# XiSHEN0220/RANSAC-Flow

Measured on NVIDIA H100. Metric: image-pairs/sec at 480x640, nbIter=1k RANSAC, higher is better.
Workload: dtype f32-grade: fp16 hi/lo split operands and activations (22 significand bits), 3 wgmma MMAs per MAC, fp32 accumulate; fp16-split correlation; fp32/fp64 RANSAC

## Files before the change

### ransac-flow_b200/csrc/gemm_tc.cu

```cuda
#include <cuda.h>
#include <cuda_fp16.h>

#include <climits>
#include <mutex>
#include <unordered_map>

#include "common.cuh"
#include "tc_common.cuh"

namespace rf {

constexpr int K_TF32 = 0, K_F16 = 1, K_SPLIT = 2, K_TF32X3 = 3;
constexpr int MODE_CONV = 0, MODE_CORR = 1;
constexpr int O_F32 = 0, O_F16 = 1, O_SPLIT = 2;
constexpr int WG_THREADS = 288;

struct alignas(64) WgParams {
    CUtensorMap mapA[RF_MAX_IMGS];
    CUtensorMap mapA2[RF_MAX_IMGS];
    CUtensorMap mapY[RF_MAX_IMGS];
    CUtensorMap mapR[RF_MAX_IMGS];
    CUtensorMap mapB;
    CUtensorMap mapBlo;
    int nimg;
    int ntiles;
    int tile_start[RF_MAX_IMGS + 1];
    int tiles_x[RF_MAX_IMGS];
    int tw[RF_MAX_IMGS];
// ... 2 lines not shown
    int R, S, pad, stride, Cin, Cout, relu, round_out;
    int dil;
    int kc1, stride2;
    long long plane;
    const float* bias;
    const void* residual;
    void* y;
    unsigned long long* rowbest;
    unsigned long long* colbest;
    int NA, NB;
};
static_assert(sizeof(WgParams) <= 32764, "kernel parameter space (CUDA 12.1+ large kernel parameters)");

template <int KIND, int BN, int MODE>
struct WgCfg {
    static constexpr int NPL = (KIND == K_SPLIT || KIND == K_TF32X3) ? 2 : 1;
    static constexpr int A_BYTES = NPL * TC_A_BYTES;
    static constexpr int B_PLANE = BN * 128;
    static constexpr int STAGE_BYTES = A_BYTES + NPL * B_PLANE;
    static constexpr bool ONE_CTA = MODE == MODE_CORR || NPL * BN >= 256;
    static constexpr int BUDGET = ONE_CTA ? 200 * 1024 : 100 * 1024;
    static constexpr int STAGES = BUDGET / STAGE_BYTES > 6 ? 6 : BUDGET / STAGE_BYTES;
    static constexpr int CTAS_PER_SM = ONE_CTA ? 1 : 2;
    static constexpr int SMEM_BYTES = STAGES * STAGE_BYTES + 1024  + 256 ;
    static_assert(STAGES >= 2 && SMEM_BYTES <= 227 * 1024, "shared memory");
};

__device__ __forceinline__ __half2 pack_sat(float a, float b) {
    uint32_t r;
    asm("cvt.rn.satfinite.f16x2.f32 %0, %1, %2;" : "=r"(r) : "f"(b), "f"(a));
    return *reinterpret_cast<__half2*>(&r);
}
__device__ __forceinline__ void split2(float a, float b, __half2& hi, __half2& lo) {
    hi = pack_sat(a, b);
    const float2 f = __half22float2(hi);
    lo = pack_sat((a - f.x) * 2048.f, (b - f.y) * 2048.f);
}

template <int KIND, int BN, int NACC>
__device__ __forceinline__ void mma_block(float (&acc)[NACC][BN / 2], uint32_t sa, uint32_t sb) {
// ... 1 lines not shown
#pragma unroll
    for (int k = 0; k < 4; ++k) {
        const uint64_t ah = wg_desc(sa + 32 * k), bh = wg_desc(sb + 32 * k);
        if constexpr (KIND == K_SPLIT || KIND == K_TF32X3) {
            const uint64_t al = wg_desc(sa + TC_A_BYTES + 32 * k), bl = wg_desc(sb + BN * 128 + 32 * k);
            float (&x)[BN / 2] = acc[NACC - 1];
            wgmma<TF32, BN>(x, al, bh);
            wgmma<TF32, BN>(x, ah, bl);
            wgmma<TF32, BN>(acc[0], ah, bh);
        } else {
            wgmma<TF32, BN>(acc[0], ah, bh);
        }
    }
}

template <int KIND, int BN, int MODE, int OUT>
__global__ void __launch_bounds__(WG_THREADS, WgCfg<KIND, BN, MODE>::CTAS_PER_SM)
wg_kernel(const __grid_constant__ WgParams p) {
    using Cfg = WgCfg<KIND, BN, MODE>;
    constexpr int STAGES = Cfg::STAGES;
    constexpr int BK = (KIND == K_TF32 || KIND == K_TF32X3) ? TC_BK : TC_BK_F16;
    constexpr int NACC = KIND == K_SPLIT ? 2 : 1;
    constexpr bool SLOT = MODE == MODE_CONV && OUT != O_F32;
    constexpr int BOX_BYTES = (OUT == O_SPLIT ? 2 : 1) * 128 * 128;
    static_assert(!SLOT || (BN / 64) * BOX_BYTES <= Cfg::STAGE_BYTES, "the output tile fits one stage");
    extern __shared__ uint8_t smem_raw[];
    uint8_t* smem = smem_raw + ((1024u - (smem_u32(smem_raw) & 1023u)) & 1023u);
    uint64_t* full = reinterpret_cast<uint64_t*>(smem + STAGES * Cfg::STAGE_BYTES);
    uint64_t* empty = full + STAGES;
    const int warp = threadIdx.x >> 5, lane = threadIdx.x & 31;
    const int kc = p.Cin / BK;
    const int KI = p.R * p.S * kc;

    const int t_first = MODE == MODE_CORR ? 0 : (int)blockIdx.x;
    const int t_step = MODE == MODE_CORR ? 1 : (int)gridDim.x;
    const int t_end = MODE == MODE_CORR ? 1 : p.ntiles;
    const int nt = (p.Cout + BN - 1) / BN;
    struct Tile { int img, tw, ox0, oy0, n0; };
    auto decode = [&](int t) {
        const int mtile = MODE == MODE_CORR ? (int)blockIdx.y : t / nt;
        const int ntile = MODE == MODE_CORR ? (int)blockIdx.x : t - mtile * nt;
        Tile T;
        T.img = 0;
#pragma unroll
        for (int j = 1; j < RF_MAX_IMGS; ++j) T.img += (j < p.nimg && mtile >= p.tile_start[j]) ? 1 : 0;
        const int tloc = mtile - p.tile_start[T.img];
        T.tw = p.tw[T.img];
        const int tyi = tloc / p.tiles_x[T.img], txi = tloc - tyi * p.tiles_x[T.img];
        T.ox0 = txi * T.tw;
        T.oy0 = tyi * (128 / T.tw);
        T.n0 = ntile * BN;
        return T;
    };
    auto boxes = [&](const Tile& T) { return BN == 64 || T.n0 + 64 >= p.Cout ? 1 : 2; };

    if (threadIdx.x == 0) {
        for (int s = 0; s < STAGES; ++s) { mbar_init(&full[s], 1); mbar_init(&empty[s], 256); }
        fence_barrier_init();
    }
    __syncthreads();

    if (warp == 8) {
        if (lane == 0) {
            tma_prefetch_desc(&p.mapB);
            uint32_t prefetched = 0;
            int st = 0;
            uint32_t ph = 0;
            for (int t = t_first; t < t_end; t += t_step) {
                const Tile T = decode(t);
                if (!((prefetched >> T.img) & 1u)) {
                    prefetched |= 1u << T.img;
                    tma_prefetch_desc(&p.mapA[T.img]);
                    if constexpr (SLOT) {
                        tma_prefetch_desc(&p.mapY[T.img]);
                        if (p.residual) tma_prefetch_desc(&p.mapR[T.img]);
                    }
                }
                for (int it = 0; it < KI; ++it) {
                    mbar_wait(&empty[st], ph ^ 1);
                    uint8_t* sa = smem + st * Cfg::STAGE_BYTES;
                    uint8_t* sb = sa + Cfg::A_BYTES;
                    mbar_expect_tx(&full[st], Cfg::STAGE_BYTES);
                    if constexpr (MODE == MODE_CORR) {
                        const int c0 = it * BK;
                        tma_load_3d(sa, &p.mapA[0], &full[st], c0, T.ox0, 0);
                        tma_load_3d(sa + TC_A_BYTES, &p.mapA2[0], &full[st], c0, T.ox0, 0);
                        tma_load_2d(sb, &p.mapB, &full[st], c0, T.n0);
                        tma_load_2d(sb + Cfg::B_PLANE, &p.mapBlo, &full[st], c0, T.n0);
                    } else {
                        const int tap = it / kc, cc = it - tap * kc;
                        const int r = tap / p.S, s = tap - r * p.S;
                        const int c0 = cc * BK, x = T.ox0 * p.stride + s * p.dil - p.pad, y = T.oy0 * p.stride + r * p.dil - p.pad;
                        const int kcol = tap * p.Cin + c0;
                        if constexpr (KIND == K_SPLIT) {
                            if (cc < p.kc1) tma_load_4d(sa, &p.mapA[T.img], &full[st], c0, x, y, 0);
                            else tma_load_4d(sa, &p.mapA2[T.img], &full[st], (cc - p.kc1) * BK, T.ox0 * p.stride2, T.oy0 * p.stride2, 0);
                            tma_load_3d(sb, &p.mapB, &full[st], kcol, T.n0, 0);
                        } else {
                            tma_load_3d(sa, &p.mapA[T.img], &full[st], c0, x, y);
                            tma_load_2d(sb, &p.mapB, &full[st], kcol, T.n0);
                        }
                    }
                    if (++st == STAGES) { st = 0; ph ^= 1; }
                }
                if constexpr (SLOT) {
                    mbar_wait(&empty[st], ph ^ 1);
                    if (p.residual) {
                        const int nb = boxes(T);
                        uint8_t* slot = smem + st * Cfg::STAGE_BYTES;
                        mbar_expect_tx(&full[st], nb * BOX_BYTES);
                        for (int b = 0; b < nb; ++b) {
                            if constexpr (OUT == O_SPLIT) tma_load_4d(slot + b * BOX_BYTES, &p.mapR[T.img], &full[st], T.n0 + 64 * b, T.ox0, T.oy0, 0);
                            else tma_load_3d(slot + b * BOX_BYTES, &p.mapR[T.img], &full[st], T.n0 + 64 * b, T.ox0, T.oy0);
                        }
                    } else {
                        mbar_arrive(&full[st]);
                    }
                    if (++st == STAGES) { st = 0; ph ^= 1; }
                }
            }
        }
        return;
    }

    const int g = warp >> 2;
    const int rbase = 64 * g + 16 * (warp & 3) + (lane >> 2);
    const int cbase = 2 * (lane & 3);
    auto before = [](int s) { return s == 0 ? STAGES - 1 : s - 1; };
    int st = 0;
    uint32_t ph = 0;
    bool stored = false;
    for (int t = t_first; t < t_end; t += t_step) {
        const Tile T = decode(t);
        float acc[NACC][BN / 2];
#pragma unroll
        for (int a = 0; a < NACC; ++a)
#pragma unroll
            for (int i = 0; i < BN / 2; ++i) acc[a][i] = 0.f;
        for (int it = 0; it < KI; ++it) {
            mbar_wait(&full[st], ph);
            const uint32_t sa = smem_u32(smem + st * Cfg::STAGE_BYTES);
            wg_fence();
            mma_block<KIND, BN, NACC>(acc, sa + g * (64 * 128), sa + Cfg::A_BYTES);
            wg_commit();
            wg_wait<1>();
            if (it > 0) {
                mbar_arrive(&empty[before(st)]);
            } else if (SLOT && stored) {
                if (threadIdx.x == 0) bulk_wait_read();
                mbar_arrive(&empty[before(st)]);
            }
            if (++st == STAGES) { st = 0; ph ^= 1; }
        }
        wg_wait<0>();
#pragma unroll
        for (int a = 0; a < NACC; ++a) wg_fence_regs(acc[a]);
        mbar_arrive(&empty[before(st)]);

        auto value = [&](int i) -> float {
            if constexpr (KIND == K_SPLIT) return fmaf(acc[1][i], 0.00048828125f, acc[0][i]);
            else return acc[0][i];
        };

        if constexpr (SLOT) {
            mbar_wait(&full[st], ph);
            uint8_t* slot = smem + st * Cfg::STAGE_BYTES;
#pragma unroll
            for (int h = 0; h < 2; ++h) {
                const int m = rbase + 8 * h;
#pragma unroll
                for (int j = 0; j < BN / 8; ++j) {
                    const int c = 8 * j + cbase, n = T.n0 + c;
                    if (n >= p.Cout) continue;
                    float v0 = value(4 * j + 2 * h), v1 = value(4 * j + 2 * h + 1);
                    if (p.bias) { v0 += __ldg(p.bias + n); v1 += __ldg(p.bias + n + 1); }
                    uint8_t* e = slot + (c >> 6) * BOX_BYTES + m * 128 + ((((c & 63) >> 3) ^ (m & 7)) << 4) + (c & 7) * 2;
                    if (p.residual) {
                        if constexpr (OUT == O_F16) {
                            const float2 r = __half22float2(*reinterpret_cast<const __half2*>(e));
                            v0 += r.x; v1 += r.y;
                        } else {
// ... 12 lines not shown
                        *reinterpret_cast<__half2*>(e + 128 * 128) = lo;
                    }
                }
            }
            fence_proxy_async();
            asm volatile("bar.sync 1, 256;" ::: "memory");
            if (threadIdx.x == 0) {
                const int nb = boxes(T);
                for (int b = 0; b < nb; ++b) {
                    if constexpr (OUT == O_SPLIT) tma_store_4d(&p.mapY[T.img], slot + b * BOX_BYTES, T.n0 + 64 * b, T.ox0, T.oy0, 0);
                    else tma_store_3d(&p.mapY[T.img], slot + b * BOX_BYTES, T.n0 + 64 * b, T.ox0, T.oy0);
                }
                bulk_commit();
            }
            stored = true;
            if (++st == STAGES) { st = 0; ph ^= 1; }
        } else if constexpr (MODE == MODE_CONV) {
            const int img = T.img, tw = T.tw;
#pragma unroll
            for (int h = 0; h < 2; ++h) {
                const int m = rbase + 8 * h;
                const int py = m / tw, px = m - py * tw;
                const int oy = T.oy0 + py, ox = T.ox0 + px;
                if (oy >= p.Ho[img] || ox >= p.Wo[img]) continue;
                const long long pix = p.out_pix[img] + (long long)oy * p.Wo[img] + ox;
#pragma unroll
                for (int j = 0; j < BN / 8; ++j) {
                    const int n = T.n0 + 8 * j + cbase;
                    if (n >= p.Cout) continue;
                    const bool two = n + 1 < p.Cout;
                    float v0 = value(4 * j + 2 * h), v1 = value(4 * j + 2 * h + 1);
                    if (p.bias) { v0 += __ldg(p.bias + n); if (two) v1 += __ldg(p.bias + n + 1); }
// ... 103 lines not shown
    int Hs[RF_MAX_IMGS], Ws[RF_MAX_IMGS];
    int Ho[RF_MAX_IMGS], Wo[RF_MAX_IMGS];
    long long in_pix[RF_MAX_IMGS], out_pix[RF_MAX_IMGS];
    long long plane;
    const float* x;
    const float* bias;
    __half* y;
};

__device__ __forceinline__ uint32_t stem_pack_split(float v) {
    __half2 hi, lo;
    split2(v, 0.f, hi, lo);
    return (*reinterpret_cast<uint32_t*>(&hi) & 0xFFFFu) | (*reinterpret_cast<uint32_t*>(&lo) << 16);
}

struct StemFrag { uint32_t h[4], l[4]; };

template <int KK, int j>
__device__ __forceinline__ void stem_gather(StemFrag& f, const uint32_t* __restrict__ w, int base, const int4* sK, int q) {
    const int4 o4 = sK[j * 4 + q];
    const int o[4] = {o4.x, o4.y, o4.z, o4.w};
    uint32_t v[2][4];
#pragma unroll
    for (int h = 0; h < 2; ++h)
#pragma unroll
        for (int e = 0; e < 4; ++e) v[h][e] = (16 * (j + 1) <= KK || o[e] >= 0) ? w[base + 24 * h + o[e]] : 0u;
#pragma unroll
    for (int e = 0; e < 2; ++e)
#pragma unroll
        for (int h = 0; h < 2; ++h) {
            f.h[2 * e + h] = __byte_perm(v[h][2 * e], v[h][2 * e + 1], 0x5410);
            f.l[2 * e + h] = __byte_perm(v[h][2 * e], v[h][2 * e + 1], 0x7632);
        }
}

template <int KK, int KSTEPS, bool SPLIT, int j, int NACC>
__device__ __forceinline__ void stem_mma(float (&acc)[NACC][32], StemFrag (&buf)[2], const uint32_t* w, int base, const int4* sK, int q,
                                         uint32_t sB) {
    if constexpr (j < KSTEPS) {
        constexpr int NPL = SPLIT ? 2 : 1;
        StemFrag& f = buf[j & 1];
        wg_fence();
        const uint32_t b = sB + (j >> 2) * NPL * ST_B_PLANE + 32 * (j & 3);
        const uint64_t bh = wg_desc(b);
        if constexpr (SPLIT) {
            wgmma_f16_n64_rs(acc[1], f.l, bh);
            wgmma_f16_n64_rs(acc[1], f.h, wg_desc(b + ST_B_PLANE));
        }
        wgmma_f16_n64_rs(acc[0], f.h, bh);
        wg_commit();
        if constexpr (j + 1 < KSTEPS) {
            wg_wait<1>();
            stem_gather<KK, j + 1>(buf[(j + 1) & 1], w, base, sK, q);
        }
        stem_mma<KK, KSTEPS, SPLIT, j + 1>(acc, buf, w, base, sK, q, sB);
    }
// ... 83 lines not shown
    stage_window(sIn);
    __syncthreads();

    const int q = lane & 3;
    const int rbase = 64 * g + 16 * (warp & 3) + (lane >> 2), cbase = 2 * q;
    const int base = (rbase >> 5) * S * G::LD + 3 * (rbase & 31);
    const uint32_t sB32 = smem_u32(sB);
    int wb = 0, tb = 0;
    for (bool first = true; u < u_end; ++u, first = false) {
        const uint32_t* w = sIn + wb * G::WIN;
        float acc[NACC][32];
#pragma unroll
        for (int a = 0; a < NACC; ++a)
#pragma unroll
            for (int i = 0; i < 32; ++i) acc[a][i] = 0.f;
        StemFrag frag[2];
        stem_gather<G::KK, 0>(frag[0], w, base, sK, q);
        if (first) mbar_wait(bar_b, 0);
        stem_mma<G::KK, G::KSTEPS, SPLIT, 0>(acc, frag, w, base, sK, q, sB32);
        const bool more = u + 1 < u_end;
        Unit N = U;
        if (more) {
            N = decode(u + 1);
            load_window(N);
        }
        wg_wait<0>();
#pragma unroll
        for (int a = 0; a < NACC; ++a) wg_fence_regs(acc[a]);

        const int img = U.img;
        uint8_t* tile = sT + tb * ST_T_BYTES;
// ... 184 lines not shown
    return get_map4(out, ptr, d0, d1, d2, 0, 0, b0, b1, b2, 0, es_, esize);
}

int pick_tw(int Ho, int Wo) {
    int best = 16;
    long long best_area = -1;
    const int cands[5] = {16, 32, 8, 64, 128};
    for (int i = 0; i < 5; ++i) {
        int tw = cands[i], th = 128 / tw;
        long long area = (long long)((Wo + tw - 1) / tw) * ((Ho + th - 1) / th);
        if (best_area < 0 || area < best_area) { best_area = area; best = tw; }
    }
    return best;
}

template <int KIND, int BN, int MODE, int OUT>
static int launch_wg(const WgParams& p, dim3 grid, cudaStream_t st) {
    using Cfg = WgCfg<KIND, BN, MODE>;
    static bool attr[64] = {false};
    const int dev = current_device();
    if (!attr[dev]) {
        RF_CUDA(cudaFuncSetAttribute(wg_kernel<KIND, BN, MODE, OUT>, cudaFuncAttributeMaxDynamicSharedMemorySize, Cfg::SMEM_BYTES));
        attr[dev] = true;
    }
    wg_kernel<KIND, BN, MODE, OUT><<<grid, WG_THREADS, Cfg::SMEM_BYTES, st>>>(p);
    RF_LAUNCHED();
    return 0;
}

template <int KIND, int BN, int OUT>
static int launch_conv_bn(const WgParams& p, cudaStream_t st) {
    const int resident = WgCfg<KIND, BN, MODE_CONV>::CTAS_PER_SM * num_sms();
    return launch_wg<KIND, BN, MODE_CONV, OUT>(p, dim3(p.ntiles < resident ? p.ntiles : resident), st);
}
template <int KIND, int OUT>
static int launch_conv(const WgParams& p, int BN, cudaStream_t st) {
    return BN == 128 ? launch_conv_bn<KIND, 128, OUT>(p, st) : launch_conv_bn<KIND, 64, OUT>(p, st);
}

struct SplitDual { const void* x2; const int* hw2; int Cin2, stride2; };

static int conv_impl(const ImgSet& batch, const ConvParams& cp, const void* w, cudaStream_t st, int kind, bool out32, const SplitDual* dual) {
    const bool flat = cp.R == 1 && cp.S == 1 && cp.stride == 1 && cp.pad == 0 && (dual == nullptr || dual->stride2 == 1);
    int hw_flat[2] = {1, 0};
    ImgSet flat_set;
    if (flat) {
        RF_REQUIRE(batch.out_pix[batch.n] <= INT_MAX, "rf_conv2d_nhwc: more than 2^31 - 1 pixels in one batch");
        hw_flat[1] = (int)batch.out_pix[batch.n];
        RF_REQUIRE(make_imgset(flat_set, 1, hw_flat, 1, 1, 0) == 0, "rf_conv2d_nhwc: bad image set");
    }
    const ImgSet& set = flat ? flat_set : batch;
    const int* hw2 = dual == nullptr ? nullptr : flat ? hw_flat : dual->hw2;
    WgParams p;
    memset(&p, 0, sizeof(p));
    const bool split = kind == K_SPLIT;
    const unsigned esz = kind == K_TF32 ? 4u : 2u;
    const unsigned bk = kind == K_TF32 ? TC_BK : TC_BK_F16;
    const int BN = cp.Cout > 64 ? 128 : 64;
    const char* xb = reinterpret_cast<const char*>(cp.x);
    const unsigned long long in_plane = (unsigned long long)set.in_pix[set.n] * cp.Cin * 2ull;
    long long in2_pix[RF_MAX_IMGS + 1] = {0};
    if (dual)
        for (int i = 0; i < set.n; ++i) in2_pix[i + 1] = in2_pix[i] + (long long)hw2[2 * i] * hw2[2 * i + 1];
    const unsigned long long in2_plane = dual ? (unsigned long long)in2_pix[set.n] * dual->Cin2 * 2ull : 0ull;
    p.nimg = set.n;
    const bool tma_out = kind != K_TF32 && !out32;
    const unsigned long long out_plane = (unsigned long long)set.out_pix[set.n] * cp.Cout * 2ull;
    const char* yb = reinterpret_cast<const char*>(cp.y);
    const char* rb = reinterpret_cast<const char*>(cp.residual);
    int tiles = 0;
    for (int i = 0; i < set.n; ++i) {
        const int tw = flat ? 128 : pick_tw(set.Ho[i], set.Wo[i]), th = 128 / tw;
        p.tw[i] = tw;
        p.tiles_x[i] = (set.Wo[i] + tw - 1) / tw;
        p.tile_start[i] = tiles;
        tiles += p.tiles_x[i] * ((set.Ho[i] + th - 1) / th);
        p.Ho[i] = set.Ho[i]; p.Wo[i] = set.Wo[i];
        p.out_pix[i] = set.out_pix[i];
        int rc = split ? get_map4(&p.mapA[i], xb + set.in_pix[i] * cp.Cin * 2, (unsigned long long)cp.Cin, (unsigned long long)set.W[i],
                                  (unsigned long long)set.H[i], 2, in_plane, bk, (unsigned)tw, (unsigned)th, 2, (unsigned)cp.stride, 2)
                       : get_map(&p.mapA[i], xb + set.in_pix[i] * cp.Cin * esz, (unsigned long long)cp.Cin, (unsigned long long)set.W[i],
                                 (unsigned long long)set.H[i], bk, (unsigned)tw, (unsigned)th, (unsigned)cp.stride, esz);
        if (!rc && dual)
            rc = get_map4(&p.mapA2[i], static_cast<const char*>(dual->x2) + in2_pix[i] * dual->Cin2 * 2, (unsigned long long)dual->Cin2,
                          (unsigned long long)hw2[2 * i + 1], (unsigned long long)hw2[2 * i], 2, in2_plane, bk, (unsigned)tw,
                          (unsigned)th, 2, (unsigned)dual->stride2, 2);
        const long long o = set.out_pix[i] * cp.Cout * 2;
        for (int m = 0; m < (cp.residual ? 2 : 1) && tma_out && !rc; ++m) {
            CUtensorMap* map = m == 0 ? &p.mapY[i] : &p.mapR[i];
            const void* base = (m == 0 ? yb : rb) + o;
            rc = split ? get_map4(map, base, (unsigned long long)cp.Cout, (unsigned long long)set.Wo[i], (unsigned long long)set.Ho[i], 2,
                                  out_plane, 64, (unsigned)tw, (unsigned)th, 2, 1, 2)
                       : get_map(map, base, (unsigned long long)cp.Cout, (unsigned long long)set.Wo[i], (unsigned long long)set.Ho[i],
                                 64, (unsigned)tw, (unsigned)th, 1, 2);
        }
        if (rc) return rc;
    }
    RF_REQUIRE(tiles > 0, "rf_conv2d_nhwc: empty output");
    for (int i = set.n; i <= RF_MAX_IMGS; ++i) p.tile_start[i] = tiles;
    p.out_pix[set.n] = set.out_pix[set.n];
    int rc = split ? get_map(&p.mapB, w, (unsigned long long)cp.K, (unsigned long long)cp.Cout, 2, bk, (unsigned)BN, 2, 1, 2)
                   : get_map(&p.mapB, w, (unsigned long long)cp.K, (unsigned long long)cp.Cout, 0, bk, (unsigned)BN, 0, 1, esz);
    if (rc) return rc;
    p.R = cp.R; p.S = cp.S; p.pad = cp.pad; p.stride = cp.stride; p.Cin = cp.Cin; p.Cout = cp.Cout; p.relu = cp.relu; p.round_out = cp.round_out;
    p.dil = cp.dil;
    p.kc1 = cp.Cin / (int)bk;
    p.stride2 = 1;
    if (dual) { p.Cin = cp.Cin + dual->Cin2; p.stride2 = dual->stride2; }
    p.plane = (long long)set.out_pix[set.n] * cp.Cout;
    p.bias = cp.bias; p.residual = cp.residual; p.y = cp.y;
    p.ntiles = tiles * ((cp.Cout + BN - 1) / BN);
    if (kind == K_TF32) return launch_conv<K_TF32, O_F32>(p, BN, st);
    if (kind == K_F16) return out32 ? launch_conv<K_F16, O_F32>(p, BN, st) : launch_conv<K_F16, O_F16>(p, BN, st);
    return out32 ? launch_conv<K_SPLIT, O_F32>(p, BN, st) : launch_conv<K_SPLIT, O_SPLIT>(p, BN, st);
}

template <int KS, int S, bool SPLIT>
static int stem_impl(const float* x, int nimg, const int* hw_host, const void* w, const float* bias, void* y, int pool, void* stream) {
    using G = StemGeo<KS, S>;
    RF_REQUIRE(x != nullptr && w != nullptr && y != nullptr, "rf_stem: null pointer");
    RF_REQUIRE(((uintptr_t)y % 16) == 0 && ((uintptr_t)w % 16) == 0, "rf_stem: pointers must be 16-byte aligned");
    ImgSet set;
    RF_REQUIRE(make_imgset(set, nimg, hw_host, KS, S, G::PAD) == 0, "rf_stem: bad image set");
    StemParams p;
    memset(&p, 0, sizeof(p));
    p.nimg = nimg;
    p.pool = pool ? 1 : 0;
    int units = 0;
    long long out = 0;
// ... 155 lines not shown
```

### ransac-flow_b200/csrc/tc_common.cuh

```cuda
#pragma once
#include <cuda.h>
#include <cuda_fp16.h>

#include "common.cuh"
#include "wgmma.cuh"

namespace rf {

constexpr int TC_BK = 32;
constexpr int TC_BK_F16 = 64;
constexpr int TC_A_BYTES = 128 * 128;


__device__ __forceinline__ uint32_t smem_u32(const void* p) { return (uint32_t)__cvta_generic_to_shared(p); }

__device__ __forceinline__ void mbar_init(uint64_t* bar, uint32_t count) {
    asm volatile("mbarrier.init.shared::cta.b64 [%0], %1;" ::"r"(smem_u32(bar)), "r"(count));
}
__device__ __forceinline__ void mbar_expect_tx(uint64_t* bar, uint32_t bytes) {
    asm volatile("mbarrier.arrive.expect_tx.shared::cta.b64 _, [%0], %1;" ::"r"(smem_u32(bar)), "r"(bytes) : "memory");
}
__device__ __forceinline__ void mbar_arrive(uint64_t* bar) {
    asm volatile("mbarrier.arrive.shared::cta.b64 _, [%0];" ::"r"(smem_u32(bar)) : "memory");
}
// ... 36 lines not shown
__device__ __forceinline__ void bulk_commit() { asm volatile("cp.async.bulk.commit_group;" ::: "memory"); }
__device__ __forceinline__ void bulk_wait_read() { asm volatile("cp.async.bulk.wait_group.read 0;" ::: "memory"); }
__device__ __forceinline__ void bulk_wait() { asm volatile("cp.async.bulk.wait_group 0;" ::: "memory"); }
__device__ __forceinline__ void tma_prefetch_desc(const CUtensorMap* map) {
    asm volatile("prefetch.tensormap [%0];" ::"l"((uint64_t)map) : "memory");
}

__device__ __forceinline__ uint64_t wg_desc(uint32_t saddr) {
    uint64_t d = 0;
    d |= (uint64_t)((saddr & 0x3FFFFu) >> 4);
    d |= (uint64_t)1 << 16;
    d |= (uint64_t)(1024 >> 4) << 32;
    d |= (uint64_t)1 << 62;
    return d;
}
__device__ __forceinline__ void wg_fence() { asm volatile("wgmma.fence.sync.aligned;" ::: "memory"); }
__device__ __forceinline__ void wg_commit() { asm volatile("wgmma.commit_group.sync.aligned;" ::: "memory"); }
template <int N>
__device__ __forceinline__ void wg_wait() { asm volatile("wgmma.wait_group.sync.aligned %0;" ::"n"(N) : "memory"); }
template <int N>
__device__ __forceinline__ void wg_fence_regs(float (&d)[N]) {
#pragma unroll
    for (int i = 0; i < N; ++i) asm volatile("" : "+f"(d[i])::"memory");
}

int get_map(CUtensorMap* out, const void* ptr, unsigned long long d0, unsigned long long d1, unsigned long long d2,
            unsigned b0, unsigned b1, unsigned b2, unsigned es_ = 1, unsigned esize = 4);
int get_map4(CUtensorMap* out, const void* ptr, unsigned long long d0, unsigned long long d1, unsigned long long d2, unsigned long long d3,
             unsigned long long plane_bytes, unsigned b0, unsigned b1, unsigned b2, unsigned b3, unsigned es_, unsigned esize);
int pick_tw(int Ho, int Wo);
// ... 3 lines not shown
```

### ransac-flow_b200/csrc/wgmma.cuh

```cuda
#pragma once
#include <stdint.h>

namespace rf {

__device__ __forceinline__ void wgmma_f16_n64(float (&d)[32], uint64_t a, uint64_t b) {
    asm volatile(
        "{\n\t.reg .pred p;\n\tsetp.ne.b32 p, 1, 0;\n\t"
        "wgmma.mma_async.sync.aligned.m64n64k16.f32.f16.f16 {%0, %1, %2, %3, %4, %5, %6, %7, %8, %9, %10, %11, %12, %13, %14, %15, %16, %17, %18, %19, %20, %21, %22, %23, %24, %25, %26, %27, %28, %29, %30, %31}, %32, %33, p, 1, 1, 0, 0;\n\t}"
        : "+f"(d[0]), "+f"(d[1]), "+f"(d[2]), "+f"(d[3]), "+f"(d[4]), "+f"(d[5]), "+f"(d[6]), "+f"(d[7]), "+f"(d[8]), "+f"(d[9]), "+f"(d[10]), "+f"(d[11]), "+f"(d[12]), "+f"(d[13]), "+f"(d[14]), "+f"(d[15]), "+f"(d[16]), "+f"(d[17]), "+f"(d[18]), "+f"(d[19]), "+f"(d[20]), "+f"(d[21]), "+f"(d[22]), "+f"(d[23]), "+f"(d[24]), "+f"(d[25]), "+f"(d[26]), "+f"(d[27]), "+f"(d[28]), "+f"(d[29]), "+f"(d[30]), "+f"(d[31])
        : "l"(a), "l"(b));
}

__device__ __forceinline__ void wgmma_f16_n128(float (&d)[64], uint64_t a, uint64_t b) {
    asm volatile(
        "{\n\t.reg .pred p;\n\tsetp.ne.b32 p, 1, 0;\n\t"
        "wgmma.mma_async.sync.aligned.m64n128k16.f32.f16.f16 {%0, %1, %2, %3, %4, %5, %6, %7, %8, %9, %10, %11, %12, %13, %14, %15, %16, %17, %18, %19, %20, %21, %22, %23, %24, %25, %26, %27, %28, %29, %30, %31, %32, %33, %34, %35, %36, %37, %38, %39, %40, %41, %42, %43, %44, %45, %46, %47, %48, %49, %50, %51, %52, %53, %54, %55, %56, %57, %58, %59, %60, %61, %62, %63}, %64, %65, p, 1, 1, 0, 0;\n\t}"
        : "+f"(d[0]), "+f"(d[1]), "+f"(d[2]), "+f"(d[3]), "+f"(d[4]), "+f"(d[5]), "+f"(d[6]), "+f"(d[7]), "+f"(d[8]), "+f"(d[9]), "+f"(d[10]), "+f"(d[11]), "+f"(d[12]), "+f"(d[13]), "+f"(d[14]), "+f"(d[15]), "+f"(d[16]), "+f"(d[17]), "+f"(d[18]), "+f"(d[19]), "+f"(d[20]), "+f"(d[21]), "+f"(d[22]), "+f"(d[23]), "+f"(d[24]), "+f"(d[25]), "+f"(d[26]), "+f"(d[27]), "+f"(d[28]), "+f"(d[29]), "+f"(d[30]), "+f"(d[31]), "+f"(d[32]), "+f"(d[33]), "+f"(d[34]), "+f"(d[35]), "+f"(d[36]), "+f"(d[37]), "+f"(d[38]), "+f"(d[39]), "+f"(d[40]), "+f"(d[41]), "+f"(d[42]), "+f"(d[43]), "+f"(d[44]), "+f"(d[45]), "+f"(d[46]), "+f"(d[47]), "+f"(d[48]), "+f"(d[49]), "+f"(d[50]), "+f"(d[51]), "+f"(d[52]), "+f"(d[53]), "+f"(d[54]), "+f"(d[55]), "+f"(d[56]), "+f"(d[57]), "+f"(d[58]), "+f"(d[59]), "+f"(d[60]), "+f"(d[61]), "+f"(d[62]), "+f"(d[63])
        : "l"(a), "l"(b));
}

__device__ __forceinline__ void wgmma_tf32_n64(float (&d)[32], uint64_t a, uint64_t b) {
    asm volatile(
        "{\n\t.reg .pred p;\n\tsetp.ne.b32 p, 1, 0;\n\t"
        "wgmma.mma_async.sync.aligned.m64n64k8.f32.tf32.tf32 {%0, %1, %2, %3, %4, %5, %6, %7, %8, %9, %10, %11, %12, %13, %14, %15, %16, %17, %18, %19, %20, %21, %22, %23, %24, %25, %26, %27, %28, %29, %30, %31}, %32, %33, p, 1, 1;\n\t}"
// ... 5 lines not shown
    asm volatile(
        "{\n\t.reg .pred p;\n\tsetp.ne.b32 p, 1, 0;\n\t"
        "wgmma.mma_async.sync.aligned.m64n128k8.f32.tf32.tf32 {%0, %1, %2, %3, %4, %5, %6, %7, %8, %9, %10, %11, %12, %13, %14, %15, %16, %17, %18, %19, %20, %21, %22, %23, %24, %25, %26, %27, %28, %29, %30, %31, %32, %33, %34, %35, %36, %37, %38, %39, %40, %41, %42, %43, %44, %45, %46, %47, %48, %49, %50, %51, %52, %53, %54, %55, %56, %57, %58, %59, %60, %61, %62, %63}, %64, %65, p, 1, 1;\n\t}"
        : "+f"(d[0]), "+f"(d[1]), "+f"(d[2]), "+f"(d[3]), "+f"(d[4]), "+f"(d[5]), "+f"(d[6]), "+f"(d[7]), "+f"(d[8]), "+f"(d[9]), "+f"(d[10]), "+f"(d[11]), "+f"(d[12]), "+f"(d[13]), "+f"(d[14]), "+f"(d[15]), "+f"(d[16]), "+f"(d[17]), "+f"(d[18]), "+f"(d[19]), "+f"(d[20]), "+f"(d[21]), "+f"(d[22]), "+f"(d[23]), "+f"(d[24]), "+f"(d[25]), "+f"(d[26]), "+f"(d[27]), "+f"(d[28]), "+f"(d[29]), "+f"(d[30]), "+f"(d[31]), "+f"(d[32]), "+f"(d[33]), "+f"(d[34]), "+f"(d[35]), "+f"(d[36]), "+f"(d[37]), "+f"(d[38]), "+f"(d[39]), "+f"(d[40]), "+f"(d[41]), "+f"(d[42]), "+f"(d[43]), "+f"(d[44]), "+f"(d[45]), "+f"(d[46]), "+f"(d[47]), "+f"(d[48]), "+f"(d[49]), "+f"(d[50]), "+f"(d[51]), "+f"(d[52]), "+f"(d[53]), "+f"(d[54]), "+f"(d[55]), "+f"(d[56]), "+f"(d[57]), "+f"(d[58]), "+f"(d[59]), "+f"(d[60]), "+f"(d[61]), "+f"(d[62]), "+f"(d[63])
        : "l"(a), "l"(b));
}

__device__ __forceinline__ void wgmma_f16_n64_rs(float (&d)[32], const uint32_t (&a)[4], uint64_t b) {
    asm volatile(
        "{\n\t.reg .pred p;\n\tsetp.ne.b32 p, 1, 0;\n\t"
        "wgmma.mma_async.sync.aligned.m64n64k16.f32.f16.f16 {%0, %1, %2, %3, %4, %5, %6, %7, %8, %9, %10, %11, %12, %13, %14, %15, %16, %17, %18, %19, %20, %21, %22, %23, %24, %25, %26, %27, %28, %29, %30, %31}, {%32, %33, %34, %35}, %36, p, 1, 1, 0;\n\t}"
        : "+f"(d[0]), "+f"(d[1]), "+f"(d[2]), "+f"(d[3]), "+f"(d[4]), "+f"(d[5]), "+f"(d[6]), "+f"(d[7]), "+f"(d[8]), "+f"(d[9]), "+f"(d[10]), "+f"(d[11]), "+f"(d[12]), "+f"(d[13]), "+f"(d[14]), "+f"(d[15]), "+f"(d[16]), "+f"(d[17]), "+f"(d[18]), "+f"(d[19]), "+f"(d[20]), "+f"(d[21]), "+f"(d[22]), "+f"(d[23]), "+f"(d[24]), "+f"(d[25]), "+f"(d[26]), "+f"(d[27]), "+f"(d[28]), "+f"(d[29]), "+f"(d[30]), "+f"(d[31])
        : "r"(a[0]), "r"(a[1]), "r"(a[2]), "r"(a[3]), "l"(b));
}

template <bool TF32, int N>
__device__ __forceinline__ void wgmma(float (&d)[N / 2], uint64_t a, uint64_t b) {
    if constexpr (TF32) { if constexpr (N == 64) wgmma_tf32_n64(d, a, b); else wgmma_tf32_n128(d, a, b); }
    else { if constexpr (N == 64) wgmma_f16_n64(d, a, b); else wgmma_f16_n128(d, a, b); }
}

}
```

Baseline: 158.6.

## Add halo-tile mode for 3x3 stride-1 convs with register-sourced wgmma

Adds a MODE_HALO path for 3x3, stride-1, pad-1 convolutions with a single input-channel chunk. It loads one halo tile of (tw+2)x(th+2) pixels per channel chunk via TMA and reuses it for all nine taps, using ldmatrix into registers and register-A wgmma. Before, the kernel reloaded a shifted A tile from global memory for every tap, so this targets A-operand load traffic and TMA issue overhead. In exchange it adds extra barriers, a separate output slot and a different tile-width heuristic, reduces pipeline stages, and moves A-fragment loads into the consumer warps, which raises register pressure.

```diff
diff --git a/ransac-flow_b200/csrc/gemm_tc.cu b/ransac-flow_b200/csrc/gemm_tc.cu
--- a/ransac-flow_b200/csrc/gemm_tc.cu
+++ b/ransac-flow_b200/csrc/gemm_tc.cu
@@ -11,7 +11,7 @@
 namespace rf {
 
 constexpr int K_TF32 = 0, K_F16 = 1, K_SPLIT = 2, K_TF32X3 = 3;
-constexpr int MODE_CONV = 0, MODE_CORR = 1;
+constexpr int MODE_CONV = 0, MODE_CORR = 1, MODE_HALO = 2;
 constexpr int O_F32 = 0, O_F16 = 1, O_SPLIT = 2;
 constexpr int WG_THREADS = 288;
 
@@ -44,16 +44,26 @@
 
 template <int KIND, int BN, int MODE>
 struct WgCfg {
+    static constexpr bool HALO = MODE == MODE_HALO;
     static constexpr int NPL = (KIND == K_SPLIT || KIND == K_TF32X3) ? 2 : 1;
-    static constexpr int A_BYTES = NPL * TC_A_BYTES;
+    static constexpr int A_BYTES = HALO ? 0 : NPL * TC_A_BYTES;
     static constexpr int B_PLANE = BN * 128;
     static constexpr int STAGE_BYTES = A_BYTES + NPL * B_PLANE;
-    static constexpr bool ONE_CTA = MODE == MODE_CORR || NPL * BN >= 256;
-    static constexpr int BUDGET = ONE_CTA ? 200 * 1024 : 100 * 1024;
+    static constexpr bool ONE_CTA = MODE == MODE_CORR || NPL * BN >= 256 || (HALO && NPL * BN >= 128);
+    static constexpr int CTAS_PER_SM = ONE_CTA ? 1 : 2;
+    static constexpr int HALO_ROWS = HALO ? 204 : 0;
+    static constexpr int TW_MAX = 32;
+    static constexpr int H_PLANE = (HALO_ROWS * 128 + 1023) / 1024 * 1024;
+    static constexpr int H_BYTES = NPL * H_PLANE;
+    static constexpr int SLOT_BYTES = HALO ? (BN / 64) * NPL * 128 * 128 : 0;
+    static constexpr int H_BUDGET = (ONE_CTA ? 227 * 1024 : 228 * 1024 / 2 - 1024) - 1280 - SLOT_BYTES;
+    static constexpr int NH = !HALO ? 0 : H_BUDGET - 2 * H_BYTES >= 2 * STAGE_BYTES ? 2 : 1;
+    static constexpr int RING_OFF = NH * H_BYTES + SLOT_BYTES;
+    static constexpr int BUDGET = HALO ? H_BUDGET - NH * H_BYTES : ONE_CTA ? 200 * 1024 : 100 * 1024;
     static constexpr int STAGES = BUDGET / STAGE_BYTES > 6 ? 6 : BUDGET / STAGE_BYTES;
-    static constexpr int CTAS_PER_SM = ONE_CTA ? 1 : 2;
-    static constexpr int SMEM_BYTES = STAGES * STAGE_BYTES + 1024  + 256 ;
+    static constexpr int SMEM_BYTES = RING_OFF + STAGES * STAGE_BYTES + 1024  + 256 ;
     static_assert(STAGES >= 2 && SMEM_BYTES <= 227 * 1024, "shared memory");
+    static_assert(!HALO || CTAS_PER_SM * (SMEM_BYTES + 1024) <= 228 * 1024, "halo mode: CTAs per SM");
 };
 
 __device__ __forceinline__ __half2 pack_sat(float a, float b) {
@@ -85,6 +95,18 @@
     }
 }
 
+struct AFrag { uint32_t h[4], l[4]; };
+
+template <int KIND, int BN, int NACC>
+__device__ __forceinline__ void mma_rs(float (&acc)[NACC][BN / 2], const AFrag& f, uint32_t sb) {
+    const uint64_t bh = wg_desc(sb);
+    if constexpr (KIND == K_SPLIT) {
+        wgmma_rs<BN>(acc[1], f.l, bh);
+        wgmma_rs<BN>(acc[1], f.h, wg_desc(sb + BN * 128));
+    }
+    wgmma_rs<BN>(acc[0], f.h, bh);
+}
+
 template <int KIND, int BN, int MODE, int OUT>
 __global__ void __launch_bounds__(WG_THREADS, WgCfg<KIND, BN, MODE>::CTAS_PER_SM)
 wg_kernel(const __grid_constant__ WgParams p) {
@@ -92,13 +114,20 @@
     constexpr int STAGES = Cfg::STAGES;
     constexpr int BK = (KIND == K_TF32 || KIND == K_TF32X3) ? TC_BK : TC_BK_F16;
     constexpr int NACC = KIND == K_SPLIT ? 2 : 1;
-    constexpr bool SLOT = MODE == MODE_CONV && OUT != O_F32;
+    constexpr bool HALO = MODE == MODE_HALO;
+    static_assert(!HALO || KIND == K_F16 || KIND == K_SPLIT, "halo mode: fp16 operand kinds");
+    constexpr bool SLOT = MODE != MODE_CORR && OUT != O_F32;
     constexpr int BOX_BYTES = (OUT == O_SPLIT ? 2 : 1) * 128 * 128;
-    static_assert(!SLOT || (BN / 64) * BOX_BYTES <= Cfg::STAGE_BYTES, "the output tile fits one stage");
+    static_assert(!SLOT || (BN / 64) * BOX_BYTES <= (HALO ? Cfg::SLOT_BYTES : Cfg::STAGE_BYTES), "the output tile fits one stage / the slot");
     extern __shared__ uint8_t smem_raw[];
     uint8_t* smem = smem_raw + ((1024u - (smem_u32(smem_raw) & 1023u)) & 1023u);
-    uint64_t* full = reinterpret_cast<uint64_t*>(smem + STAGES * Cfg::STAGE_BYTES);
+    uint8_t* ring = smem + Cfg::RING_OFF;
+    uint64_t* full = reinterpret_cast<uint64_t*>(ring + STAGES * Cfg::STAGE_BYTES);
     uint64_t* empty = full + STAGES;
+    uint64_t* hfull = empty + STAGES;
+    uint64_t* hempty = hfull + 2;
+    uint64_t* sfull = hfull + 4;
+    uint64_t* sempty = hfull + 5;
     const int warp = threadIdx.x >> 5, lane = threadIdx.x & 31;
     const int kc = p.Cin / BK;
     const int KI = p.R * p.S * kc;
@@ -127,6 +156,11 @@
 
     if (threadIdx.x == 0) {
         for (int s = 0; s < STAGES; ++s) { mbar_init(&full[s], 1); mbar_init(&empty[s], 256); }
+        if constexpr (HALO) {
+            for (int h = 0; h < Cfg::NH; ++h) { mbar_init(&hfull[h], 1); mbar_init(&hempty[h], 256); }
+            mbar_init(sfull, 1);
+            mbar_init(sempty, 1);
+        }
         fence_barrier_init();
     }
     __syncthreads();
@@ -135,8 +169,8 @@
         if (lane == 0) {
             tma_prefetch_desc(&p.mapB);
             uint32_t prefetched = 0;
-            int st = 0;
-            uint32_t ph = 0;
+            int st = 0, hs = 0;
+            uint32_t ph = 0, hph = 0, sph = 0;
             for (int t = t_first; t < t_end; t += t_step) {
                 const Tile T = decode(t);
                 if (!((prefetched >> T.img) & 1u)) {
@@ -147,9 +181,33 @@
                         if (p.residual) tma_prefetch_desc(&p.mapR[T.img]);
                     }
                 }
-                for (int it = 0; it < KI; ++it) {
+                if constexpr (HALO) {
+                    const uint32_t hbytes = Cfg::NPL * (T.tw + 2) * (128 / T.tw + 2) * 128;
+                    for (int cc = 0; cc < kc; ++cc) {
+                        mbar_wait(&hempty[hs], hph ^ 1);
+                        mbar_expect_tx(&hfull[hs], hbytes);
+                        uint8_t* hb = smem + hs * Cfg::H_BYTES;
+                        if constexpr (KIND == K_SPLIT) {
+                            tma_load_4d(hb, &p.mapA[T.img], &hfull[hs], cc * BK, T.ox0 - 1, T.oy0 - 1, 0);
+                            tma_load_4d(hb + Cfg::H_PLANE, &p.mapA[T.img], &hfull[hs], cc * BK, T.ox0 - 1, T.oy0 - 1, 1);
+                        } else {
+                            tma_load_3d(hb, &p.mapA[T.img], &hfull[hs], cc * BK, T.ox0 - 1, T.oy0 - 1);
+                        }
+                        if (++hs == Cfg::NH) { hs = 0; hph ^= 1; }
+                        for (int tap = 0; tap < 9; ++tap) {
+                            mbar_wait(&empty[st], ph ^ 1);
+                            uint8_t* sb = ring + st * Cfg::STAGE_BYTES;
+                            mbar_expect_tx(&full[st], Cfg::STAGE_BYTES);
+                            const int kcol = tap * p.Cin + cc * BK;
+                            if constexpr (KIND == K_SPLIT) tma_load_3d(sb, &p.mapB, &full[st], kcol, T.n0, 0);
+                            else tma_load_2d(sb, &p.mapB, &full[st], kcol, T.n0);
+                            if (++st == STAGES) { st = 0; ph ^= 1; }
+                        }
+                    }
+                }
+                for (int it = 0; it < (HALO ? 0 : KI); ++it) {
                     mbar_wait(&empty[st], ph ^ 1);
-                    uint8_t* sa = smem + st * Cfg::STAGE_BYTES;
+                    uint8_t* sa = ring + st * Cfg::STAGE_BYTES;
                     uint8_t* sb = sa + Cfg::A_BYTES;
                     mbar_expect_tx(&full[st], Cfg::STAGE_BYTES);
                     if constexpr (MODE == MODE_CORR) {
@@ -175,19 +233,21 @@
                     if (++st == STAGES) { st = 0; ph ^= 1; }
                 }
                 if constexpr (SLOT) {
-                    mbar_wait(&empty[st], ph ^ 1);
+                    uint64_t* sf = HALO ? sfull : &full[st];
+                    mbar_wait(HALO ? sempty : &empty[st], (HALO ? sph : ph) ^ 1);
                     if (p.residual) {
                         const int nb = boxes(T);
-                        uint8_t* slot = smem + st * Cfg::STAGE_BYTES;
-                        mbar_expect_tx(&full[st], nb * BOX_BYTES);
+                        uint8_t* slot = HALO ? ring - Cfg::SLOT_BYTES : ring + st * Cfg::STAGE_BYTES;
+                        mbar_expect_tx(sf, nb * BOX_BYTES);
                         for (int b = 0; b < nb; ++b) {
-                            if constexpr (OUT == O_SPLIT) tma_load_4d(slot + b * BOX_BYTES, &p.mapR[T.img], &full[st], T.n0 + 64 * b, T.ox0, T.oy0, 0);
-                            else tma_load_3d(slot + b * BOX_BYTES, &p.mapR[T.img], &full[st], T.n0 + 64 * b, T.ox0, T.oy0);
+                            if constexpr (OUT == O_SPLIT) tma_load_4d(slot + b * BOX_BYTES, &p.mapR[T.img], sf, T.n0 + 64 * b, T.ox0, T.oy0, 0);
+                            else tma_load_3d(slot + b * BOX_BYTES, &p.mapR[T.img], sf, T.n0 + 64 * b, T.ox0, T.oy0);
                         }
                     } else {
-                        mbar_arrive(&full[st]);
+                        mbar_arrive(sf);
                     }
-                    if (++st == STAGES) { st = 0; ph ^= 1; }
+                    if constexpr (HALO) sph ^= 1;
+                    else if (++st == STAGES) { st = 0; ph ^= 1; }
                 }
             }
         }
@@ -198,9 +258,11 @@
     const int rbase = 64 * g + 16 * (warp & 3) + (lane >> 2);
     const int cbase = 2 * (lane & 3);
     auto before = [](int s) { return s == 0 ? STAGES - 1 : s - 1; };
-    int st = 0;
-    uint32_t ph = 0;
+    int st = 0, hs = 0;
+    uint32_t ph = 0, hph = 0, sph = 0;
     bool stored = false;
+    const int lrow = 64 * g + 16 * (warp & 3) + (lane & 7) + (lane & 8), lk = lane >> 4;
+    const uint32_t sh = smem_u32(smem);
     for (int t = t_first; t < t_end; t += t_step) {
         const Tile T = decode(t);
         float acc[NACC][BN / 2];
@@ -208,9 +270,54 @@
         for (int a = 0; a < NACC; ++a)
 #pragma unroll
             for (int i = 0; i < BN / 2; ++i) acc[a][i] = 0.f;
-        for (int it = 0; it < KI; ++it) {
+        if constexpr (HALO) {
+            const int hw = T.tw + 2, py = lrow / T.tw, r0 = py * hw + lrow - py * T.tw;
+            for (int cc = 0; cc < kc; ++cc) {
+                AFrag f[2];
+                uint32_t hb;
+                asm volatile("mov.b32 %0, %1;" : "=r"(hb) : "r"(sh + hs * Cfg::H_BYTES));
+                auto load = [&](AFrag& f, int row, int k) {
+                    const uint32_t a = hb + row * 128 + (((2 * k + lk) ^ (row & 7)) << 4);
+                    ldsm_x4(f.h, a);
+                    if constexpr (KIND == K_SPLIT) ldsm_x4(f.l, a + Cfg::H_PLANE);
+                };
+                mbar_wait(&hfull[hs], hph);
+                load(f[0], r0, 0);
+#pragma unroll
+                for (int tap = 0; tap < 9; ++tap) {
+                    const int row = r0 + (tap / 3) * hw + tap % 3;
+                    mbar_wait(&full[st], ph);
+                    const uint32_t sb = smem_u32(ring + st * Cfg::STAGE_BYTES);
+#pragma unroll
+                    for (int k = 0; k < 4; ++k) {
+                        wg_fence();
+                        mma_rs<KIND, BN, NACC>(acc, f[k & 1], sb + 32 * k);
+                        wg_commit();
+                        wg_wait<1>();
+                        if (k == 0 && tap > 0) {
+                            mbar_arrive(&empty[before(st)]);
+                        } else if (k == 0 && cc == 0 && SLOT && stored && threadIdx.x == 0) {
+                            bulk_wait_read();
+                            mbar_arrive(sempty);
+                        }
+                        if (k < 3) {
+                            load(f[(k + 1) & 1], row, k + 1);
+                        } else if (tap < 8) {
+                            load(f[0], row + (tap % 3 == 2 ? hw - 2 : 1), 0);
+                        } else {
+                            mbar_arrive(&hempty[hs]);
+                            if (++hs == Cfg::NH) { hs = 0; hph ^= 1; }
+                        }
+                    }
+                    if (++st == STAGES) { st = 0; ph ^= 1; }
+                }
+                wg_wait<0>();
+                mbar_arrive(&empty[before(st)]);
+            }
+        }
+        for (int it = 0; it < (HALO ? 0 : KI); ++it) {
             mbar_wait(&full[st], ph);
-            const uint32_t sa = smem_u32(smem + st * Cfg::STAGE_BYTES);
+            const uint32_t sa = smem_u32(ring + st * Cfg::STAGE_BYTES);
             wg_fence();
             mma_block<KIND, BN, NACC>(acc, sa + g * (64 * 128), sa + Cfg::A_BYTES);
             wg_commit();
@@ -226,7 +333,7 @@
         wg_wait<0>();
 #pragma unroll
         for (int a = 0; a < NACC; ++a) wg_fence_regs(acc[a]);
-        mbar_arrive(&empty[before(st)]);
+        if constexpr (!HALO) mbar_arrive(&empty[before(st)]);
 
         auto value = [&](int i) -> float {
             if constexpr (KIND == K_SPLIT) return fmaf(acc[1][i], 0.00048828125f, acc[0][i]);
@@ -234,8 +341,8 @@
         };
 
         if constexpr (SLOT) {
-            mbar_wait(&full[st], ph);
-            uint8_t* slot = smem + st * Cfg::STAGE_BYTES;
+            mbar_wait(HALO ? sfull : &full[st], HALO ? sph : ph);
+            uint8_t* slot = HALO ? ring - Cfg::SLOT_BYTES : ring + st * Cfg::STAGE_BYTES;
 #pragma unroll
             for (int h = 0; h < 2; ++h) {
                 const int m = rbase + 8 * h;
@@ -278,8 +385,9 @@
                 bulk_commit();
             }
             stored = true;
-            if (++st == STAGES) { st = 0; ph ^= 1; }
-        } else if constexpr (MODE == MODE_CONV) {
+            if constexpr (HALO) sph ^= 1;
+            else if (++st == STAGES) { st = 0; ph ^= 1; }
+        } else if constexpr (MODE != MODE_CORR) {
             const int img = T.img, tw = T.tw;
 #pragma unroll
             for (int h = 0; h < 2; ++h) {
@@ -413,10 +521,8 @@
     return (*reinterpret_cast<uint32_t*>(&hi) & 0xFFFFu) | (*reinterpret_cast<uint32_t*>(&lo) << 16);
 }
 
-struct StemFrag { uint32_t h[4], l[4]; };
-
 template <int KK, int j>
-__device__ __forceinline__ void stem_gather(StemFrag& f, const uint32_t* __restrict__ w, int base, const int4* sK, int q) {
+__device__ __forceinline__ void stem_gather(AFrag& f, const uint32_t* __restrict__ w, int base, const int4* sK, int q) {
     const int4 o4 = sK[j * 4 + q];
     const int o[4] = {o4.x, o4.y, o4.z, o4.w};
     uint32_t v[2][4];
@@ -434,11 +540,11 @@
 }
 
 template <int KK, int KSTEPS, bool SPLIT, int j, int NACC>
-__device__ __forceinline__ void stem_mma(float (&acc)[NACC][32], StemFrag (&buf)[2], const uint32_t* w, int base, const int4* sK, int q,
+__device__ __forceinline__ void stem_mma(float (&acc)[NACC][32], AFrag (&buf)[2], const uint32_t* w, int base, const int4* sK, int q,
                                          uint32_t sB) {
     if constexpr (j < KSTEPS) {
         constexpr int NPL = SPLIT ? 2 : 1;
-        StemFrag& f = buf[j & 1];
+        AFrag& f = buf[j & 1];
         wg_fence();
         const uint32_t b = sB + (j >> 2) * NPL * ST_B_PLANE + 32 * (j & 3);
         const uint64_t bh = wg_desc(b);
@@ -552,7 +658,7 @@
         for (int a = 0; a < NACC; ++a)
 #pragma unroll
             for (int i = 0; i < 32; ++i) acc[a][i] = 0.f;
-        StemFrag frag[2];
+        AFrag frag[2];
         stem_gather<G::KK, 0>(frag[0], w, base, sK, q);
         if (first) mbar_wait(bar_b, 0);
         stem_mma<G::KK, G::KSTEPS, SPLIT, 0>(acc, frag, w, base, sK, q, sB32);
@@ -767,6 +873,19 @@
     return best;
 }
 
+static int pick_tw_halo(int Ho, int Wo, int tw_max, int BN) {
+    int best = 16;
+    long long best_cost = -1;
+    const int cands[3] = {16, 32, 8};
+    for (int i = 0; i < 3; ++i) {
+        const int tw = cands[i], th = 128 / tw;
+        if (tw > tw_max) continue;
+        const long long cost = (long long)((Wo + tw - 1) / tw) * ((Ho + th - 1) / th) * ((tw + 2) * (th + 2) + 9 * BN);
+        if (best_cost < 0 || cost < best_cost) { best_cost = cost; best = tw; }
+    }
+    return best;
+}
+
 template <int KIND, int BN, int MODE, int OUT>
 static int launch_wg(const WgParams& p, dim3 grid, cudaStream_t st) {
     using Cfg = WgCfg<KIND, BN, MODE>;
@@ -781,14 +900,18 @@
     return 0;
 }
 
-template <int KIND, int BN, int OUT>
+template <int KIND, int BN, int MODE, int OUT>
 static int launch_conv_bn(const WgParams& p, cudaStream_t st) {
-    const int resident = WgCfg<KIND, BN, MODE_CONV>::CTAS_PER_SM * num_sms();
-    return launch_wg<KIND, BN, MODE_CONV, OUT>(p, dim3(p.ntiles < resident ? p.ntiles : resident), st);
+    const int resident = WgCfg<KIND, BN, MODE>::CTAS_PER_SM * num_sms();
+    return launch_wg<KIND, BN, MODE, OUT>(p, dim3(p.ntiles < resident ? p.ntiles : resident), st);
 }
 template <int KIND, int OUT>
-static int launch_conv(const WgParams& p, int BN, cudaStream_t st) {
-    return BN == 128 ? launch_conv_bn<KIND, 128, OUT>(p, st) : launch_conv_bn<KIND, 64, OUT>(p, st);
+static int launch_conv(const WgParams& p, int BN, bool halo, cudaStream_t st) {
+    if constexpr (KIND == K_F16)
+        if (halo) return BN == 128 ? launch_conv_bn<KIND, 128, MODE_HALO, OUT>(p, st) : launch_conv_bn<KIND, 64, MODE_HALO, OUT>(p, st);
+    if constexpr (KIND == K_SPLIT)
+        if (halo) return launch_conv_bn<KIND, 64, MODE_HALO, OUT>(p, st);
+    return BN == 128 ? launch_conv_bn<KIND, 128, MODE_CONV, OUT>(p, st) : launch_conv_bn<KIND, 64, MODE_CONV, OUT>(p, st);
 }
 
 struct SplitDual { const void* x2; const int* hw2; int Cin2, stride2; };
@@ -810,6 +933,9 @@
     const unsigned esz = kind == K_TF32 ? 4u : 2u;
     const unsigned bk = kind == K_TF32 ? TC_BK : TC_BK_F16;
     const int BN = cp.Cout > 64 ? 128 : 64;
+    const bool halo = kind != K_TF32 && cp.R == 3 && cp.S == 3 && cp.stride == 1 && cp.pad == 1 && cp.dil == 1 && dual == nullptr &&
+                      cp.Cin == (int)bk && !(split && BN == 128);
+    const int tw_max = WgCfg<K_F16, 64, MODE_HALO>::TW_MAX;
     const char* xb = reinterpret_cast<const char*>(cp.x);
     const unsigned long long in_plane = (unsigned long long)set.in_pix[set.n] * cp.Cin * 2ull;
     long long in2_pix[RF_MAX_IMGS + 1] = {0};
@@ -823,17 +949,18 @@
     const char* rb = reinterpret_cast<const char*>(cp.residual);
     int tiles = 0;
     for (int i = 0; i < set.n; ++i) {
-        const int tw = flat ? 128 : pick_tw(set.Ho[i], set.Wo[i]), th = 128 / tw;
+        const int tw = flat ? 128 : halo ? pick_tw_halo(set.Ho[i], set.Wo[i], tw_max, BN) : pick_tw(set.Ho[i], set.Wo[i]), th = 128 / tw;
         p.tw[i] = tw;
         p.tiles_x[i] = (set.Wo[i] + tw - 1) / tw;
         p.tile_start[i] = tiles;
         tiles += p.tiles_x[i] * ((set.Ho[i] + th - 1) / th);
         p.Ho[i] = set.Ho[i]; p.Wo[i] = set.Wo[i];
         p.out_pix[i] = set.out_pix[i];
+        const unsigned bw = halo ? tw + 2 : tw, bh = halo ? th + 2 : th;
         int rc = split ? get_map4(&p.mapA[i], xb + set.in_pix[i] * cp.Cin * 2, (unsigned long long)cp.Cin, (unsigned long long)set.W[i],
-                                  (unsigned long long)set.H[i], 2, in_plane, bk, (unsigned)tw, (unsigned)th, 2, (unsigned)cp.stride, 2)
+                                  (unsigned long long)set.H[i], 2, in_plane, bk, bw, bh, halo ? 1 : 2, (unsigned)cp.stride, 2)
                        : get_map(&p.mapA[i], xb + set.in_pix[i] * cp.Cin * esz, (unsigned long long)cp.Cin, (unsigned long long)set.W[i],
-                                 (unsigned long long)set.H[i], bk, (unsigned)tw, (unsigned)th, (unsigned)cp.stride, esz);
+                                 (unsigned long long)set.H[i], bk, bw, bh, (unsigned)cp.stride, esz);
         if (!rc && dual)
             rc = get_map4(&p.mapA2[i], static_cast<const char*>(dual->x2) + in2_pix[i] * dual->Cin2 * 2, (unsigned long long)dual->Cin2,
                           (unsigned long long)hw2[2 * i + 1], (unsigned long long)hw2[2 * i], 2, in2_plane, bk, (unsigned)tw,
@@ -863,9 +990,9 @@
     p.plane = (long long)set.out_pix[set.n] * cp.Cout;
     p.bias = cp.bias; p.residual = cp.residual; p.y = cp.y;
     p.ntiles = tiles * ((cp.Cout + BN - 1) / BN);
-    if (kind == K_TF32) return launch_conv<K_TF32, O_F32>(p, BN, st);
-    if (kind == K_F16) return out32 ? launch_conv<K_F16, O_F32>(p, BN, st) : launch_conv<K_F16, O_F16>(p, BN, st);
-    return out32 ? launch_conv<K_SPLIT, O_F32>(p, BN, st) : launch_conv<K_SPLIT, O_SPLIT>(p, BN, st);
+    if (kind == K_TF32) return launch_conv<K_TF32, O_F32>(p, BN, false, st);
+    if (kind == K_F16) return out32 ? launch_conv<K_F16, O_F32>(p, BN, halo, st) : launch_conv<K_F16, O_F16>(p, BN, halo, st);
+    return out32 ? launch_conv<K_SPLIT, O_F32>(p, BN, halo, st) : launch_conv<K_SPLIT, O_SPLIT>(p, BN, halo, st);
 }
 
 template <int KS, int S, bool SPLIT>
diff --git a/ransac-flow_b200/csrc/tc_common.cuh b/ransac-flow_b200/csrc/tc_common.cuh
--- a/ransac-flow_b200/csrc/tc_common.cuh
+++ b/ransac-flow_b200/csrc/tc_common.cuh
@@ -74,6 +74,10 @@
     d |= (uint64_t)1 << 62;
     return d;
 }
+__device__ __forceinline__ void ldsm_x4(uint32_t (&r)[4], uint32_t saddr) {
+    asm volatile("ldmatrix.sync.aligned.m8n8.x4.shared.b16 {%0, %1, %2, %3}, [%4];"
+                 : "=r"(r[0]), "=r"(r[1]), "=r"(r[2]), "=r"(r[3]) : "r"(saddr) : "memory");
+}
 __device__ __forceinline__ void wg_fence() { asm volatile("wgmma.fence.sync.aligned;" ::: "memory"); }
 __device__ __forceinline__ void wg_commit() { asm volatile("wgmma.commit_group.sync.aligned;" ::: "memory"); }
 template <int N>
diff --git a/ransac-flow_b200/csrc/wgmma.cuh b/ransac-flow_b200/csrc/wgmma.cuh
--- a/ransac-flow_b200/csrc/wgmma.cuh
+++ b/ransac-flow_b200/csrc/wgmma.cuh
@@ -43,6 +43,19 @@
         : "r"(a[0]), "r"(a[1]), "r"(a[2]), "r"(a[3]), "l"(b));
 }
 
+__device__ __forceinline__ void wgmma_f16_n128_rs(float (&d)[64], const uint32_t (&a)[4], uint64_t b) {
+    asm volatile(
+        "{\n\t.reg .pred p;\n\tsetp.ne.b32 p, 1, 0;\n\t"
+        "wgmma.mma_async.sync.aligned.m64n128k16.f32.f16.f16 {%0, %1, %2, %3, %4, %5, %6, %7, %8, %9, %10, %11, %12, %13, %14, %15, %16, %17, %18, %19, %20, %21, %22, %23, %24, %25, %26, %27, %28, %29, %30, %31, %32, %33, %34, %35, %36, %37, %38, %39, %40, %41, %42, %43, %44, %45, %46, %47, %48, %49, %50, %51, %52, %53, %54, %55, %56, %57, %58, %59, %60, %61, %62, %63}, {%64, %65, %66, %67}, %68, p, 1, 1, 0;\n\t}"
+        : "+f"(d[0]), "+f"(d[1]), "+f"(d[2]), "+f"(d[3]), "+f"(d[4]), "+f"(d[5]), "+f"(d[6]), "+f"(d[7]), "+f"(d[8]), "+f"(d[9]), "+f"(d[10]), "+f"(d[11]), "+f"(d[12]), "+f"(d[13]), "+f"(d[14]), "+f"(d[15]), "+f"(d[16]), "+f"(d[17]), "+f"(d[18]), "+f"(d[19]), "+f"(d[20]), "+f"(d[21]), "+f"(d[22]), "+f"(d[23]), "+f"(d[24]), "+f"(d[25]), "+f"(d[26]), "+f"(d[27]), "+f"(d[28]), "+f"(d[29]), "+f"(d[30]), "+f"(d[31]), "+f"(d[32]), "+f"(d[33]), "+f"(d[34]), "+f"(d[35]), "+f"(d[36]), "+f"(d[37]), "+f"(d[38]), "+f"(d[39]), "+f"(d[40]), "+f"(d[41]), "+f"(d[42]), "+f"(d[43]), "+f"(d[44]), "+f"(d[45]), "+f"(d[46]), "+f"(d[47]), "+f"(d[48]), "+f"(d[49]), "+f"(d[50]), "+f"(d[51]), "+f"(d[52]), "+f"(d[53]), "+f"(d[54]), "+f"(d[55]), "+f"(d[56]), "+f"(d[57]), "+f"(d[58]), "+f"(d[59]), "+f"(d[60]), "+f"(d[61]), "+f"(d[62]), "+f"(d[63])
+        : "r"(a[0]), "r"(a[1]), "r"(a[2]), "r"(a[3]), "l"(b));
+}
+
+template <int N>
+__device__ __forceinline__ void wgmma_rs(float (&d)[N / 2], const uint32_t (&a)[4], uint64_t b) {
+    if constexpr (N == 64) wgmma_f16_n64_rs(d, a, b); else wgmma_f16_n128_rs(d, a, b);
+}
+
 template <bool TF32, int N>
 __device__ __forceinline__ void wgmma(float (&d)[N / 2], uint64_t a, uint64_t b) {
     if constexpr (TF32) { if constexpr (N == 64) wgmma_tf32_n64(d, a, b); else wgmma_tf32_n128(d, a, b); }
```

Result: faster. 160.7, median of 6 (+1.3%).
